# songhayeong/aes-fhe

Hardware: AMD Instinct MI355X
Metric: AES-128 blocks/sec (homomorphic full round) at N=2^16, L=30; 1/2/4/8 MI355X (higher is better)
Workload: dtype u64

## Files before the change

### aes-fhe_amd/csrc/engine.hip

```cpp
#include <hip/hip_runtime.h>

#include <algorithm>
#include <atomic>
#include <cstdarg>
#include <cstdlib>
#include <cstdio>
#include <cstring>
#include <map>
#include <unordered_map>
#include <memory>
#include <mutex>
#include <string>
#include <vector>

#include "../../include/aesfhe.h"
#include "kernels_ops.h"
#include "ntt256f.h"
#include "ks_fused.h"
#include "bconv_mfma.h"
#include "bconv_cols.h"
#include "basis_tables.h"
#include "bsgs_plan.h"
#include "operands.h"
#include "arena.h"
// ... 77 lines not shown
    }
    void split(void* p, int parts, size_t part) {
        if (!Arena::split(p, parts, part))
            throw_err(AESFHE_EARG, "pool split of a block that is not %d x %zu bytes", parts, part);
        if (trace) fprintf(trace, "s %c %p %d %zu\n", tag, p, parts, part);
    }
};

struct HipFree {
    void operator()(void* p) const { hipFree(p); }
};
struct DevBlocks {
    std::vector<std::unique_ptr<void, HipFree>> blocks;
    void* get(size_t bytes) {
        blocks.reserve(blocks.size() + 1);
        void* p = nullptr;
        HIPC(hipMalloc(&p, std::max<size_t>(bytes, 8)));
        blocks.emplace_back(p);
        return p;
    }
    template <typename T>
    T* up(const std::vector<T>& v) {
        T* d = (T*)get(v.size() * sizeof(T));
        HIPC(hipMemcpy(d, v.data(), v.size() * sizeof(T), hipMemcpyHostToDevice));
        return d;
    }
    void drop(void* p) {
        blocks.erase(std::remove_if(blocks.begin(), blocks.end(), [p](const auto& b) { return b.get() == p; }), blocks.end());
    }
};

struct ProfRec {
    int fam;
    hipEvent_t a, b;
    double bytes;
    const char* label;
    int disp;
};

struct KernStat {
    int64_t n = 0, d = 0;
    double ms = 0, bytes = 0;
};

struct MdTabs {
    const double *invf, *ninvf, *einv;
    const int8_t* tab;
    const double* corr;
    const u64* dinv;
    const double* dinvf;
    const TwD* hatf;
    const double* dmodf;
};

struct aesfhe_engine {
    std::atomic<int> refs{1};
    int logN, N, L, K, A, dnum, np, Lp1;
    int device = 0;
    u64 seed;
    ChaKey ck;
    Chain chain;
    hipStream_t stream = nullptr;
    Pool pool, tpool;
    size_t peak_total = 0;
    DevBlocks dev;
    u64* q;
    double* qinv;
    Tabs tab{};
    std::vector<u64> h_iroot;
    double *mu_hatinvf, *mu_nhatf, *rs_invf;
    MdTabs md;
    u64 *pmod, *rs_inv, *rs_mod;
    const double* pmodf;
    int8_t* bc_mu_tab;
    double *bc_mu_corr, *bc_pc;
    char* ring_d = nullptr;
    char* ring_h = nullptr;
    size_t ring_size = 8u << 20, ring_off = 0;
    double *ckre = nullptr, *ckim = nullptr;
    long* crot = nullptr;
    int* cflags = nullptr;
    size_t cflags_n = 0;
    std::map<std::string, TwD*> poly2_tabs;
    int prof = 0;
    std::vector<ProfRec> recs;
    std::vector<hipEvent_t> spare;
    double prof_ms[4] = {0, 0, 0, 0};
    double prof_bytes[4] = {0, 0, 0, 0};
    int64_t prof_n[4] = {0, 0, 0, 0};
    std::map<std::string, KernStat> prof_k;

    const Tabs& tabs() const { return tab; }

    ~aesfhe_engine() {
        if (!stream) return;
        hipSetDevice(device);
        hipStreamSynchronize(stream);
        for (auto& r : recs) {
            hipEventDestroy(r.a);
            hipEventDestroy(r.b);
        }
        for (auto ev : spare) hipEventDestroy(ev);
        pool.release_all();
        tpool.release_all();
        if (pool.trace) fclose(pool.trace);
        for (auto& kv : poly2_tabs) hipFree(kv.second);
        if (ring_d) hipFree(ring_d);
        if (ring_h) hipHostFree(ring_h);
        hipStreamDestroy(stream);
    }
};

struct aesfhe_key {
    aesfhe_engine* eng;
    int kind;
    u64 galois;
    u64 keyseed;
    u64* d;
    size_t bytes;
    int ndig = 0;
};

struct aesfhe_ct {
    aesfhe_engine* eng;
    int B, np, level, is_zero;
    u64* d;
    size_t bytes;
};

struct aesfhe_pt {
    aesfhe_engine* eng;
    int level;
    int ext = 0;
    u64* d;
    size_t bytes;
};

static const int FAM_NTT = 0, FAM_KS = 1, FAM_EW = 2;

struct ProfScope {
    aesfhe_engine* e;
    int fam;
    double bytes;
    hipEvent_t a = nullptr, b = nullptr;
    hipStream_t s;
    bool on;
    const char* label;
    int disp = 1;
    ProfScope(aesfhe_engine* e_, int f, double by, const char* lab = nullptr, hipStream_t s_ = nullptr)
        : e(e_), fam(f), bytes(by), s(s_ ? s_ : e_->stream), on((e_->prof >> f) & 1), label(lab) {
        if (!on) return;
        a = take();
        b = take();
        hipEventRecord(a, s);
    }
    hipEvent_t take() {
        if (!e->spare.empty()) {
            hipEvent_t x = e->spare.back();
            e->spare.pop_back();
            return x;
        }
        hipEvent_t x;
        hipEventCreate(&x);
        return x;
    }
    ~ProfScope() {
        if (!on) return;
        hipEventRecord(b, s);
        e->recs.push_back({fam, a, b, bytes, label, disp});
    }
};

static void prof_flush(aesfhe_engine* e) {
    if (e->recs.empty()) return;
    hipStreamSynchronize(e->stream);
    for (auto& r : e->recs) {
        float ms = 0;
        hipEventElapsedTime(&ms, r.a, r.b);
        e->prof_ms[r.fam] += ms;
        e->prof_bytes[r.fam] += r.bytes;
        e->prof_n[r.fam] += 1;
        if (r.label) {
            KernStat& k = e->prof_k[r.label];
            k.n++;
            k.d += r.disp;
            k.ms += ms;
            k.bytes += r.bytes;
        }
        e->spare.push_back(r.a);
// ... 2663 lines not shown
        const long obs = 3L * nl * N;
        d3 = ct_new(e, Bt, 3, l);
        {
            ProfScope ps_(e, FAM_EW, 8.0 * N * nl * (double)B * (2.0 * (nx + ny - 2) + 3.0 * ml), "poly2");
            for (int t0 = 0; t0 < ml; t0 += kPoly2Out)
                hipLaunchKernelGGL(k_poly2, ew_grid(e, nl, B), dim3(256), 0, e->stream, d[0].ptr, d[0].bs, d[0].ps, nx, d[1].ptr, d[1].bs, d[1].ps, ny, tab, ml, t0, std::min(kPoly2Out, ml - t0), d3->d, (long)B * obs, obs, e->q, e->qinv, e->logN);
        }
        HIPC(hipGetLastError());
    }
    poly2_finish(e, std::move(d3), rlk, live, m, B, l, outs);
    API_END
}

static void poly2_int_impl(aesfhe_engine* e, const aesfhe_ct* const* xb, int32_t nx, const aesfhe_ct* const* yb,
                           int32_t ny, const int32_t* w, int32_t den, int32_t m, const aesfhe_key* rlk,
                           aesfhe_ct** outs, int slab_rot);
extern "C" int aesfhe_poly2_int(aesfhe_engine* e, const aesfhe_ct* const* xb, int32_t nx, const aesfhe_ct* const* yb, int32_t ny, const int32_t* w, int32_t den, int32_t m, const aesfhe_key* rlk, aesfhe_ct** outs) {
    API_BEGIN
    poly2_int_impl(e, xb, nx, yb, ny, w, den, m, rlk, outs, 0);
    API_END
}
extern "C" int aesfhe_poly2_int_rot(aesfhe_engine* e, const aesfhe_ct* const* xb, int32_t nx, const aesfhe_ct* const* yb, int32_t ny, const int32_t* w, int32_t den, int32_t m, const aesfhe_key* rlk, int32_t slab_rot, aesfhe_ct** outs) {
    API_BEGIN
    if (slab_rot < 0 || slab_rot > 3) throw_err(AESFHE_EARG, "slab rotation %d outside 0..3", slab_rot);
    poly2_int_impl(e, xb, nx, yb, ny, w, den, m, rlk, outs, slab_rot);
    API_END
}
static void poly2_int_impl(aesfhe_engine* e, const aesfhe_ct* const* xb, int32_t nx, const aesfhe_ct* const* yb,
                           int32_t ny, const int32_t* w, int32_t den, int32_t m, const aesfhe_key* rlk,
                           aesfhe_ct** outs, int slab_rot) {
    const OperandScan sc = poly2_check(xb, nx, yb, ny, m, rlk, den);
    const int l = sc.level, B = sc.B;
    if (slab_rot && B % 4) throw_err(AESFHE_EARG, "slab rotation needs a batch of whole slabs (4 s), got %d", B);
    double wfac = 1.0;
    for (int t = 0; t < m; t++)
        for (int i = 0; i < nx; i++) {
            long sum = 0;
            double f = 0.0;
            for (int j = 0; j < ny; j++) {
                const long a = std::labs((long)w[((size_t)t * nx + i) * ny + j]);
                sum += a;
                f += j == 0 ? (double)a : 0.5 * (double)a + 1e-3 * (double)a;
            }
            if (sum > 512) throw_err(AESFHE_EARG, "poly2_int: sum of |w| over a row exceeds 512");
            wfac = std::max(wfac, f);
        }
    const int nl = l + 1, N = e->N;
    const double* D = e->chain.scale.data();
    const double S1 = D[l - 2] / D[l] * ((double)e->chain.q[l] / D[l]) * (double)e->chain.q[l - 1];
    const int64_t R = llround(D[l]);
    auto classes = [&](const aesfhe_ct* const* b, int n, std::vector<int>& cls, std::vector<int>& lev) {
        lev.clear();
        for (int i = 0; i < n - 1; i++)
            if (std::find(lev.begin(), lev.end(), b[i]->level) == lev.end()) lev.push_back(b[i]->level);
        std::sort(lev.rbegin(), lev.rend());
        cls.assign(n, 0);
        for (int i = 1; i < n; i++) cls[i] = 1 + (int)(std::find(lev.begin(), lev.end(), b[i - 1]->level) - lev.begin());
    };
    std::vector<int> cx, cy0, lx, ly;
    classes(xb, nx, cx, lx);
    classes(yb, ny, cy0, ly);
    std::vector<int> perm(ny), permx(nx);
    for (int j = 0; j < ny; j++) perm[j] = j;
    for (int i = 0; i < nx; i++) permx[i] = i;
    std::stable_sort(perm.begin() + 1, perm.end(), [&](int a, int b) { return cy0[a] < cy0[b]; });
    std::stable_sort(permx.begin() + 1, permx.end(), [&](int a, int b) { return cx[a] < cx[b]; });
    std::vector<int> cy(ny), cxs(nx);
    for (int j = 0; j < ny; j++) cy[j] = cy0[perm[j]];
    for (int i = 0; i < nx; i++) cxs[i] = cx[permx[i]];
    const int cxn = 1 + (int)lx.size(), cyn = 1 + (int)ly.size();
    std::vector<int> live;
    std::vector<double> Wt;
    for (int t = 0; t < m; t++) {
        bool any = false;
        for (size_t c = 0; c < (size_t)nx * ny; c++) any |= w[(size_t)t * nx * ny + c] != 0;
        if (!any) continue;
        live.push_back(t);
        for (int i = 0; i < nx; i++)
            for (int j = 0; j < ny; j++) Wt.push_back((double)w[((size_t)t * nx + permx[i]) * ny + perm[j]]);
    }
    const int ml = (int)live.size();
    CtPtr d3;
    if (ml > 0) {
        std::vector<TwD> Rt((size_t)nl * cxn * cyn);
        std::vector<double> C0((size_t)nl * cxn);
        for (int li = 0; li < nl; li++) {
            const u64 q = e->chain.q[li];
            const u64 r1 = h_smod(R, q);
            std::vector<u64> H((size_t)cxn * cyn);
            for (int a = 0; a < cxn; a++)
                for (int b = 0; b < cyn; b++) {
                    const double rx = a == 0 ? 1.0 : D[l] / D[lx[a - 1]];
                    const double ry = b == 0 ? 1.0 : D[l] / D[ly[b - 1]];
                    u64 h = h_smod(llround(S1 * rx * ry / (double)den), q);
                    if (a == 0) h = h_mulmod(h, r1, q);
                    if (b == 0) h = h_mulmod(h, r1, q);
                    H[(size_t)a * cyn + b] = h;
                }
            for (int a = 0; a < cxn; a++) {
                C0[(size_t)li * cxn + a] = (double)H[(size_t)a * cyn];
                for (int b = 0; b < cyn; b++) {
                    const u64 v = H[(size_t)a * cyn + b];
                    Rt[((size_t)li * cxn + a) * cyn + b] = TwD{(double)v, (double)v / (double)q};
                }
            }
        }
        const OperandTable tx = poly2_basis(xb, nx, permx.data(), B), ty = poly2_basis(yb, ny, perm.data(), B);
        const auto d = upload(e, {&tx, &ty}, OP_PTR | OP_BS | OP_PS);
        std::vector<int> xstart(cxn + 1, nx);
        for (int i = nx - 1; i >= 0; i--) xstart[cxs[i]] = i;
        auto dcx = upload_small(e, xstart.data(), xstart.size());
        auto dcy = upload_small(e, cy.data(), cy.size());
        auto dW = upload_small(e, Wt.data(), Wt.size());
        auto dR = upload_small(e, Rt.data(), Rt.size());
        auto dC0 = upload_small(e, C0.data(), C0.size());
        const long obs = 3L * nl * N;
        d3 = ct_new(e, ml * B, 3, l);
        auto is_big = [&](int li) {
            const double q = (double)e->chain.q[li];
            return wfac * q >= 0x1p52 * 0.999 || (wfac + 3.0 * nx) * q >= 0x1p53 * 0.999;
        };
        double wfac_u = 1.0;
        for (int t = 0; t < ml; t++)
            for (int i = 0; i < nx; i++) {
                double f = 0.0;
                for (int j = 0; j < ny; j++) f += std::fabs(Wt[((size_t)t * nx + i) * ny + j]);
                wfac_u = std::max(wfac_u, f);
            }
        auto lazy_ok = [&](int li) {
            const double q = (double)e->chain.q[li];
            return wfac_u * q < 0x1p51 && (wfac_u + 3.0 * nx) * q < 0x1p52;
        };
        {
            ProfScope ps_(e, FAM_EW, 8.0 * N * nl * (double)B * (2.0 * (nx + ny - 2) + 3.0 * ml), "poly2_int");
            ps_.disp = 0;
            constexpr int mo = 4;
            for (int t0 = 0; t0 < ml;) {
                const bool sbox = ny == kPoly2Max && ml - t0 >= 2 * mo && (N / 256) % 8 == 0;
                for (int la = 0; la < nl;) {
                    const bool big = is_big(la), lz = !big && lazy_ok(la);
                    int lb = la + 1;
                    while (lb < nl && is_big(lb) == big && (big || lazy_ok(lb) == lz)) lb++;
                    const dim3 grid(N / 256, lb - la, B);
                    bool split = big;
                    for (int li = la; li < lb; li++) split &= (double)e->chain.q[li] < 0x1p51;
                    if (sbox && split) {
                        hipLaunchKernelGGL(k_poly2_int_split<mo>, dim3(2 * N / 256, lb - la, B), dim3(256), 0, e->stream,
                                           d[0].ptr, d[0].bs, d[0].ps, nx, d[1].ptr, d[1].bs, d[1].ps,
                                           (const int*)dcx, (const int*)dcy, cxn, cyn, (const double*)dW, (const TwD*)dR, (const double*)dC0, t0,
                                           d3->d, (long)B * obs, obs, e->q, e->qinv, la, nl, e->logN, slab_rot);
                        ps_.disp++;
                    } else if (sbox) {
                        hipLaunchKernelGGL((big ? k_poly2_int_s<mo, false, true> : lz ? k_poly2_int_s<mo, true> : k_poly2_int_s<mo, false>), dim3(2 * N / 256, lb - la, B), dim3(256), 0, e->stream,
                                           d[0].ptr, d[0].bs, d[0].ps, nx, d[1].ptr, d[1].bs, d[1].ps,
                                           (const int*)dcx, (const int*)dcy, cxn, cyn, (const double*)dW, (const TwD*)dR, (const double*)dC0, t0,
                                           d3->d, (long)B * obs, obs, e->q, e->qinv, la, nl, e->logN, slab_rot);
                        ps_.disp++;
                    } else {
                        auto kern = big ? (ny == kPoly2Max ? k_poly2_int<true, kPoly2Max, mo> : k_poly2_int<true, 0, mo>)
                                        : (ny == kPoly2Max ? k_poly2_int<false, kPoly2Max, mo> : k_poly2_int<false, 0, mo>);
                        for (int tb = t0; tb < (sbox ? t0 + 2 * mo : t0 + mo) && tb < ml; tb += mo) {
                            hipLaunchKernelGGL(kern, grid, dim3(256), 0, e->stream, d[0].ptr, d[0].bs, d[0].ps, nx, d[1].ptr, d[1].bs, d[1].ps, ny,
                                               (const int*)dcx, (const int*)dcy, cxn, cyn, (const double*)dW, (const TwD*)dR, (const double*)dC0, ml, tb, std::min(mo, ml - tb), d3->d, (long)B * obs, obs, e->q, e->qinv, la, nl, e->logN, slab_rot);
                            ps_.disp++;
                        }
                    }
                    la = lb;
                }
                t0 += sbox ? 2 * mo : mo;
            }
        }
        HIPC(hipGetLastError());
    }
    poly2_finish(e, std::move(d3), rlk, live, m, B, l, outs);
}

extern "C" int aesfhe_ntt_host(aesfhe_engine* e, uint64_t* limbs, int32_t nlimb, const int32_t* pids, int32_t inv) {
    API_BEGIN
    const int N = e->N;
    for (int i = 0; i < nlimb; i++)
        if (pids[i] < 0 || pids[i] >= e->np) throw_err(AESFHE_EARG, "bad prime index");
    Tmp buf(e, (size_t)N);
    for (int i = 0; i < nlimb; i++) {
        HIPC(hipMemcpyAsync(buf.p, limbs + (size_t)i * N, (size_t)N * 8, hipMemcpyHostToDevice, e->stream));
        const int pid = pids[i];
        Span s = pid < e->Lp1 ? span_s(buf.p, N, 1, 1, pid, e->Lp1) : span_s(buf.p, N, 1, 0, 0, pid);
        ntt(e, s, s, 1, inv != 0);
        HIPC(hipMemcpyAsync(limbs + (size_t)i * N, buf.p, (size_t)N * 8, hipMemcpyDeviceToHost, e->stream));
        HIPC(hipStreamSynchronize(e->stream));
    }
    API_END
}

extern "C" int aesfhe_bench_ntt(aesfhe_engine* e, int32_t nlimb, int32_t iters, double* fwd_ms, double* inv_ms) {
    API_BEGIN
    const int N = e->N;
    const int nq = std::min(nlimb, e->Lp1);
    const int groups = (nlimb + nq - 1) / nq;
    Tmp buf(e, (size_t)groups * nq * N);
    HIPC(hipMemsetAsync(buf.p, 0, (size_t)groups * nq * N * 8, e->stream));
    Span s = span_s(buf.p, (long)nq * N, nq, nq, 0, e->Lp1);
    hipEvent_t a, b, c;
    HIPC(hipEventCreate(&a));
    HIPC(hipEventCreate(&b));
    HIPC(hipEventCreate(&c));
    ntt(e, s, s, groups * nq, false);
    ntt(e, s, s, groups * nq, true);
    HIPC(hipEventRecord(a, e->stream));
    for (int i = 0; i < iters; i++) ntt(e, s, s, groups * nq, false);
    HIPC(hipEventRecord(b, e->stream));
    for (int i = 0; i < iters; i++) ntt(e, s, s, groups * nq, true);
    HIPC(hipEventRecord(c, e->stream));
    HIPC(hipEventSynchronize(c));
    float t1 = 0, t2 = 0;
    hipEventElapsedTime(&t1, a, b);
    hipEventElapsedTime(&t2, b, c);
    *fwd_ms = t1 / iters;
    *inv_ms = t2 / iters;
    hipEventDestroy(a);
    hipEventDestroy(b);
    hipEventDestroy(c);
    API_END
}
```

### aes-fhe_amd/csrc/kernels_ops.h

```cpp
#pragma once
#include "kernels.h"

namespace aesfhe {

__device__ __forceinline__ u64 red_m(u64 x, u64 q, double qinv) {
    u64 qh = (u64)((double)x * qinv);
    return fix_m(x - qh * q, q);
}

struct Opnd {
    const u64* ptr;
    long bs;
    long ps;
    int np;
    int bmask = -1;
};

__device__ const u64 kZeroWord = 0;
__device__ __forceinline__ u64 opnd_get(const Opnd& o, int b, int p, int l, int k, int logN) {
    const bool has = o.ptr && p < o.np;
    return *(has ? o.ptr + (long)(b & o.bmask) * o.bs + (long)p * o.ps + ((long)l << logN) + k : &kZeroWord);
}

struct Out {
// ... 627 lines not shown
                        const long* __restrict__ ybs, const long* __restrict__ yps, int ny,
                        const TwD* __restrict__ F, int mtot, int t0, int mc,
                        u64* __restrict__ out, long oos, long obs, const u64* __restrict__ qs,
                        const double* __restrict__ qinv, int logN) {
    const int k = blockIdx.x * blockDim.x + threadIdx.x;
    const int l = blockIdx.y, bb = blockIdx.z, nl = gridDim.y;
    const int h = (int)((blockIdx.x * blockDim.x) >> (logN - 1));
    const double q = (double)qs[l];
    const double qi = qinv[l];
    const long off = ((long)l << logN) + k;
    double y0[kPoly2Max - 1], y1[kPoly2Max - 1];
#pragma unroll
    for (int j = 0; j < kPoly2Max - 1; j++) {
        y0[j] = y1[j] = 0.0;
        if (j < ny - 1) {
            const u64* p = yp[j] + (long)bb * ybs[j] + off;
            y0[j] = u2d(p[0]);
            y1[j] = u2d(p[yps[j]]);
        }
    }
    double d0[kPoly2Out], d1[kPoly2Out], d2[kPoly2Out];
#pragma unroll
    for (int t = 0; t < kPoly2Out; t++) d0[t] = d1[t] = d2[t] = 0.0;
    const TwD* Fl = F + ((size_t)(l * 2 + h) * mtot + t0) * nx * ny;
#pragma unroll 1
    for (int i = 0; i < nx; i++) {
        double xa = 0.0, xb = 0.0;
        if (i > 0) {
            const u64* p = xp[i - 1] + (long)bb * xbs[i - 1] + off;
            xa = u2d(p[0]);
            xb = u2d(p[xps[i - 1]]);
        }
#pragma unroll
        for (int t = 0; t < kPoly2Out; t++) {
            if (t < mc) {
                const TwD* Fi = Fl + ((size_t)t * nx + i) * ny;
                double a0 = Fi[0].w, a1 = 0.0;
#pragma unroll
                for (int j = 1; j < kPoly2Max; j++) {
                    if (j < ny) {
                        const TwD f = Fi[j];
                        a0 += fmul_rem_r(y0[j - 1], f.w, f.wq, q);
                        a1 += fmul_rem_r(y1[j - 1], f.w, f.wq, q);
                        if ((j & 3) == 0) {
                            a0 = fred(a0, q, qi);
                            a1 = fred(a1, q, qi);
                        }
                    }
                }
                a0 = fred(a0, q, qi);
                a1 = fred(a1, q, qi);
                if (i == 0) {
                    d0[t] += a0;
                    d1[t] += a1;
                } else {
                    const double a0q = a0 * qi, a1q = a1 * qi;
                    d0[t] += fmul_rem(xa, a0, a0q, q);
                    d1[t] += fmul_rem(xa, a1, a1q, q) + fmul_rem(xb, a0, a0q, q);
                    d2[t] += fmul_rem(xb, a1, a1q, q);
                }
                d0[t] = fred(d0[t], q, qi);
                d1[t] = fred(d1[t], q, qi);
                d2[t] = fred(d2[t], q, qi);
            }
        }
    }
    u64* o = out + (long)bb * obs + off;
    const long pstr = (long)nl << logN;
#pragma unroll
    for (int t = 0; t < kPoly2Out; t++) {
        if (t < mc) {
            u64* ot = o + (long)(t0 + t) * oos;
            ot[0] = fcanon(d0[t], q, qi);
            ot[pstr] = fcanon(d1[t], q, qi);
            ot[2 * pstr] = fcanon(d2[t], q, qi);
        }
    }
}

template <bool BIG, int NY, int MO>
__global__ void __launch_bounds__(256, MO > 4 ? 2 : 3) k_poly2_int(const u64* const* __restrict__ xp, const long* __restrict__ xbs,
                        const long* __restrict__ xps, int nx, const u64* const* __restrict__ yp,
                        const long* __restrict__ ybs, const long* __restrict__ yps, int ny,
                        const int* __restrict__ xstart, const int* __restrict__ ycls, int cxn,
                        int cyn, const double* __restrict__ Wt, const TwD* __restrict__ Rt,
                        const double* __restrict__ C0, int mtot, int t0, int mc,
                        u64* __restrict__ out, long oos, long obs, const u64* __restrict__ qs,
                        const double* __restrict__ qinv, int l0, int nl, int logN, int orot) {
    const int k = blockIdx.x * blockDim.x + threadIdx.x;
    const int l = l0 + blockIdx.y, bb = blockIdx.z;
    const double q = (double)qs[l];
    const double qi = qinv[l];
    constexpr bool big = BIG;
    const int nyv = NY > 0 ? NY : ny;
    const long off = ((long)l << logN) + k;
    double d0[MO], d1[MO], d2[MO];
#pragma unroll
    for (int t = 0; t < MO; t++) d0[t] = d1[t] = d2[t] = 0.0;
    const TwD* Rl = Rt + (size_t)l * cxn * cyn;
#pragma unroll 1
    for (int c = 0; c < cxn; c++) {
        const TwD* Rc = Rl + c * cyn;
        double y0[kPoly2Max - 1], y1[kPoly2Max - 1];
#pragma unroll
        for (int j = 0; j < kPoly2Max - 1; j++) {
            y0[j] = y1[j] = 0.0;
            if (j < nyv - 1) {
                const u64* p = yp[j] + (long)bb * ybs[j] + off;
                const TwD r = Rc[ycls[j + 1]];
                y0[j] = fred(fmul_rem_r(u2d(p[0]), r.w, r.wq, q), q, qi);
                y1[j] = fred(fmul_rem_r(u2d(p[yps[j]]), r.w, r.wq, q), q, qi);
            }
        }
        const double c0 = C0[(size_t)l * cxn + c];
#pragma unroll 1
    for (int i = xstart[c]; i < xstart[c + 1]; i++) {
        double xa = 0.0, xb = 0.0;
        if (i > 0) {
            const u64* p = xp[i - 1] + (long)bb * xbs[i - 1] + off;
            xa = u2d(p[0]);
            xb = u2d(p[xps[i - 1]]);
        }
#pragma unroll
        for (int t = 0; t < MO; t++) {
            if (t < mc) {
                const double* w = Wt + ((size_t)(t0 + t) * nx + i) * ny;
                double a0, a1;
                if constexpr (!big) {
                    a0 = w[0] * c0;
                    a1 = 0.0;
#pragma unroll
                    for (int j = 1; j < kPoly2Max; j++) {
                        if (j < nyv) {
                            a0 = __builtin_fma(w[j], y0[j - 1], a0);
                            a1 = __builtin_fma(w[j], y1[j - 1], a1);
                        }
                    }
                } else {
                    const double w0 = w[0];
                    a0 = fmul_rem(c0, w0, w0 * qi, q);
                    a1 = 0.0;
#pragma unroll
                    for (int j = 1; j < kPoly2Max; j++) {
                        if (j < nyv) {
                            const double wj = w[j], wjq = wj * qi;
                            a0 = fred(a0 + fmul_rem(y0[j - 1], wj, wjq, q), q, qi);
                            a1 = fred(a1 + fmul_rem(y1[j - 1], wj, wjq, q), q, qi);
                        }
                    }
                }
                if (i == 0) {
                    d0[t] += a0;
                    d1[t] += a1;
                } else {
                    const double a0q = a0 * qi, a1q = a1 * qi;
                    d0[t] += fmul_rem(xa, a0, a0q, q);
                    d1[t] += fmul_rem(xa, a1, a1q, q) + fmul_rem(xb, a0, a0q, q);
                    d2[t] += fmul_rem(xb, a1, a1q, q);
                }
                if constexpr (big) {
                    d0[t] = fred(d0[t], q, qi);
                    d1[t] = fred(d1[t], q, qi);
                    d2[t] = fred(d2[t], q, qi);
                }
            }
        }
    }
    }
    const int ob = (bb & ~3) | ((bb - orot) & 3);
    u64* o = out + (long)ob * obs + off;
    const long pstr = (long)nl << logN;
#pragma unroll
    for (int t = 0; t < MO; t++) {
        if (t < mc) {
            u64* ot = o + (long)(t0 + t) * oos;
            ot[0] = fcanon(d0[t], q, qi);
            ot[pstr] = fcanon(d1[t], q, qi);
            ot[2 * pstr] = fcanon(d2[t], q, qi);
        }
    }
}

template <int NY, bool BIG>
__device__ __forceinline__ void inner_sums(const double* __restrict__ w, double c0, const double (&y0)[NY - 1],
                                           const double (&y1)[NY - 1], double q, double qi, double& a0, double& a1) {
    if constexpr (!BIG) {
        a0 = w[0] * c0;
        a1 = 0.0;
#pragma unroll
        for (int j = 1; j < NY; j++) {
            a0 = __builtin_fma(w[j], y0[j - 1], a0);
            a1 = __builtin_fma(w[j], y1[j - 1], a1);
        }
    } else {
        const double w0 = w[0];
        a0 = fmul_rem(c0, w0, w0 * qi, q);
        a1 = 0.0;
#pragma unroll
        for (int j = 1; j < NY; j++) {
            const double wj = w[j], wjq = wj * qi;
            a0 = fred(a0 + fmul_rem(y0[j - 1], wj, wjq, q), q, qi);
            a1 = fred(a1 + fmul_rem(y1[j - 1], wj, wjq, q), q, qi);
        }
    }
}

template <int MO, bool LAZY, bool BIG = false>
__global__ void __launch_bounds__(256, 3) k_poly2_int_s(const u64* const* __restrict__ xp, const long* __restrict__ xbs,
                        const long* __restrict__ xps, int nx, const u64* const* __restrict__ yp,
                        const long* __restrict__ ybs, const long* __restrict__ yps,
                        const int* __restrict__ xstart, const int* __restrict__ ycls, int cxn,
                        int cyn, const double* __restrict__ Wt, const TwD* __restrict__ Rt,
                        const double* __restrict__ C0, int t0, u64* __restrict__ out, long oos, long obs,
                        const u64* __restrict__ qs, const double* __restrict__ qinv, int l0, int nl,
                        int logN, int orot) {
    constexpr int NY = kPoly2Max;
    static_assert(!(BIG && LAZY), "the folding path needs reduced y'");
    const int bx = blockIdx.x, half = (bx >> 3) & 1;
    const int k = (((bx >> 4) << 3) | (bx & 7)) * blockDim.x + threadIdx.x;
    const int l = l0 + blockIdx.y, bb = blockIdx.z;
    t0 += half * MO;
    const double q = (double)qs[l];
    const double qi = qinv[l];
    const long off = ((long)l << logN) + k;
    const TwD* Rl = Rt + (size_t)l * cxn * cyn;
    double y0[NY - 1], y1[NY - 1];
    auto load_y = [&](int c) {
        const TwD* Rc = Rl + c * cyn;
#pragma unroll
        for (int j = 0; j < NY - 1; j++) {
            const u64* p = yp[j] + (long)bb * ybs[j] + off;
            const TwD r = Rc[ycls[j + 1]];
            const double v0 = fmul_rem_r(u2d(p[0]), r.w, r.wq, q), v1 = fmul_rem_r(u2d(p[yps[j]]), r.w, r.wq, q);
            y0[j] = LAZY ? v0 : fred(v0, q, qi);
            y1[j] = LAZY ? v1 : fred(v1, q, qi);
        }
    };
    double d0[MO], d1[MO], d2[MO];
    load_y(0);
    {
        const double c0 = C0[(size_t)l * cxn];
#pragma unroll
        for (int t = 0; t < MO; t++) {
            const double* w = Wt + (size_t)(t0 + t) * nx * NY;
            double a0, a1;
            inner_sums<NY, BIG>(w, c0, y0, y1, q, qi, a0, a1);
            d0[t] = a0;
            d1[t] = a1;
            d2[t] = 0.0;
        }
    }
#pragma unroll 1
    for (int c = 1; c < cxn; c++) {
        load_y(c);
        const double c0 = C0[(size_t)l * cxn + c];
#pragma unroll 1
        for (int i = xstart[c]; i < xstart[c + 1]; i++) {
            const u64* p = xp[i - 1] + (long)bb * xbs[i - 1] + off;
            const double xa = u2d(p[0]), xb = u2d(p[xps[i - 1]]);
#pragma unroll
            for (int t = 0; t < MO; t++) {
                const double* w = Wt + ((size_t)(t0 + t) * nx + i) * NY;
                double a0, a1;
                inner_sums<NY, BIG>(w, c0, y0, y1, q, qi, a0, a1);
                const double a0q = a0 * qi, a1q = a1 * qi;
                d0[t] += fmul_rem(xa, a0, a0q, q);
                d1[t] += fmul_rem(xa, a1, a1q, q) + fmul_rem(xb, a0, a0q, q);
                d2[t] += fmul_rem(xb, a1, a1q, q);
                if constexpr (BIG) {
                    d0[t] = fred(d0[t], q, qi);
                    d1[t] = fred(d1[t], q, qi);
                    d2[t] = fred(d2[t], q, qi);
                }
            }
        }
    }
    const int ob = (bb & ~3) | ((bb - orot) & 3);
    u64* o = out + (long)ob * obs + off;
    const long pstr = (long)nl << logN;
#pragma unroll
    for (int t = 0; t < MO; t++) {
        u64* ot = o + (long)(t0 + t) * oos;
        ot[0] = fcanon(d0[t], q, qi);
        ot[pstr] = fcanon(d1[t], q, qi);
        ot[2 * pstr] = fcanon(d2[t], q, qi);
    }
}

template <int MO>
__global__ void __launch_bounds__(256, 3) k_poly2_int_split(const u64* const* __restrict__ xp, const long* __restrict__ xbs,
                        const long* __restrict__ xps, int nx, const u64* const* __restrict__ yp,
                        const long* __restrict__ ybs, const long* __restrict__ yps,
                        const int* __restrict__ xstart, const int* __restrict__ ycls, int cxn,
                        int cyn, const double* __restrict__ Wt, const TwD* __restrict__ Rt,
                        const double* __restrict__ C0, int t0, u64* __restrict__ out, long oos, long obs,
                        const u64* __restrict__ qs, const double* __restrict__ qinv, int l0, int nl,
                        int logN, int orot) {
    constexpr int NY = kPoly2Max;
    constexpr double S = 16777216.0, Si = 1.0 / 16777216.0;
    const int bx = blockIdx.x, half = (bx >> 3) & 1;
    const int k = (((bx >> 4) << 3) | (bx & 7)) * blockDim.x + threadIdx.x;
    const int l = l0 + blockIdx.y, bb = blockIdx.z;
    t0 += half * MO;
    const double q = (double)qs[l], qi = qinv[l], sq = S * qi;
    const long off = ((long)l << logN) + k;
    const TwD* Rl = Rt + (size_t)l * cxn * cyn;
    double d0[MO], d1[MO], d2[MO];
#pragma unroll
    for (int t = 0; t < MO; t++) d0[t] = d1[t] = d2[t] = 0.0;
#pragma unroll 1
    for (int p = 0; p < 2; p++) {
        double yh[NY - 1], yl[NY - 1];
#pragma unroll 1
        for (int c = 0; c < cxn; c++) {
            const TwD* Rc = Rl + c * cyn;
#pragma unroll
            for (int j = 0; j < NY - 1; j++) {
                const u64* yq = yp[j] + (long)bb * ybs[j] + off + (p ? yps[j] : 0);
                const TwD r = Rc[ycls[j + 1]];
                const double v = fred(fmul_rem_r(u2d(*yq), r.w, r.wq, q), q, qi);
                yh[j] = __builtin_rint(v * Si);
                yl[j] = __builtin_fma(-yh[j], S, v);
            }
            const double c0 = p ? 0.0 : C0[(size_t)l * cxn + c];
            const double c0h = __builtin_rint(c0 * Si), c0l = __builtin_fma(-c0h, S, c0);
#pragma unroll 1
            for (int i = xstart[c]; i < xstart[c + 1]; i++) {
                double xa = 1.0, xb = 0.0;
                if (i > 0) {
                    const u64* xq = xp[i - 1] + (long)bb * xbs[i - 1] + off;
                    xa = u2d(xq[0]);
                    xb = u2d(xq[xps[i - 1]]);
                }
#pragma unroll
                for (int t = 0; t < MO; t++) {
                    const double* w = Wt + ((size_t)(t0 + t) * nx + i) * NY;
                    double ah = w[0] * c0h, al = w[0] * c0l;
#pragma unroll
                    for (int j = 1; j < NY; j++) {
                        ah = __builtin_fma(w[j], yh[j - 1], ah);
                        al = __builtin_fma(w[j], yl[j - 1], al);
                    }
                    const double a = fmul_rem(ah, S, sq, q) + al, aq = a * qi;
                    if (i == 0) {
                        if (p == 0) d0[t] += a;
                        else d1[t] += a;
                    } else if (p == 0) {
                        d0[t] += fmul_rem(xa, a, aq, q);
                        d1[t] += fmul_rem(xb, a, aq, q);
                    } else {
                        d1[t] += fmul_rem(xa, a, aq, q);
                        d2[t] += fmul_rem(xb, a, aq, q);
                    }
                    d0[t] = fred(d0[t], q, qi);
                    d1[t] = fred(d1[t], q, qi);
                    d2[t] = fred(d2[t], q, qi);
                }
            }
        }
    }
    const int ob = (bb & ~3) | ((bb - orot) & 3);
    u64* o = out + (long)ob * obs + off;
    const long pstr = (long)nl << logN;
#pragma unroll
    for (int t = 0; t < MO; t++) {
        u64* ot = o + (long)(t0 + t) * oos;
        ot[0] = fcanon(d0[t], q, qi);
        ot[pstr] = fcanon(d1[t], q, qi);
        ot[2 * pstr] = fcanon(d2[t], q, qi);
    }
}

__global__ void k_lift0(const u64* __restrict__ x, u64* __restrict__ out, int nl, u64 q0,
                        const u64* __restrict__ qs, int logN) {
    const int k = blockIdx.x * blockDim.x + threadIdx.x;
    const int i = blockIdx.y, p = blockIdx.z;
    const u64 v = x[((long)p << logN) + k], q = qs[i];
    u64 r;
    if (v > (q0 >> 1)) {
        const u64 m = (q0 - v) % q;
        r = m ? q - m : 0;
    } else {
        r = v % q;
    }
    out[(((long)p * nl + i) << logN) + k] = r;
}

__global__ void k_dot_pt(const u64* const* __restrict__ cp, const long* __restrict__ cbs, long cps,
                         const u64* const* __restrict__ pp, int n, Out o, int np,
                         const u64* __restrict__ qs, const double* __restrict__ qinv, int logN) {
    const int k = blockIdx.x * blockDim.x + threadIdx.x;
    const int l = blockIdx.y, bb = blockIdx.z / np, p = blockIdx.z - bb * np;
    const double q = (double)qs[l], qi = qinv[l];
    const long off = ((long)l << logN) + k;
    double acc = 0.0;
    int i = 0;
    for (; i + 8 <= n; i += 8) {
        double cv[8], wv[8];
#pragma unroll
        for (int u = 0; u < 8; u++) {
            cv[u] = u2d(cp[i + u][(long)bb * cbs[i + u] + (long)p * cps + off]);
            wv[u] = u2d(pp[i + u][off]);
        }
#pragma unroll
        for (int u = 0; u < 8; u++) {
            acc += fmul_remq(cv[u], wv[u], qi, q);
            if ((u & 3) == 3) acc = fred(acc, q, qi);
        }
    }
    for (; i < n; i++) {
        const double c = u2d(cp[i][(long)bb * cbs[i] + (long)p * cps + off]);
        const double w = u2d(pp[i][off]);
        acc += fmul_remq(c, w, qi, q);
        if ((i & 3) == 3) acc = fred(acc, q, qi);
    }
    o.ptr[(long)bb * o.bs + (long)p * o.ps + off] = fcanon(acc, q, qi);
}

__device__ __forceinline__ int ext_pid(int t, int l, int Lp1) { return t <= l ? t : Lp1 + (t - l - 1); }

__global__ void k_scale_p_ext(Opnd in, u64* __restrict__ out, int l, int ne, const u64* __restrict__ qall,
                              const double* __restrict__ qinvall, const double* __restrict__ pmodf, int Lp1, int logN) {
    const int k = blockIdx.x * blockDim.x + threadIdx.x;
    const int t = blockIdx.y, bb = blockIdx.z >> 1, c = blockIdx.z & 1;
    u64 v = 0;
    if (t <= l) {
        const double q = (double)qall[t], qi = qinvall[t], f = pmodf[t];
        v = fcanon(fmul_rem(u2d(opnd_get(in, bb, c, t, k, logN)), tw_w(f, q), f, q), q, qi);
    }
    out[((((long)bb * 2 + c) * ne + t) << logN) + k] = v;
}

template <int GM, int BCT>
__global__ void k_dot_pt_ext_multi(const u64* const* __restrict__ ep, const u64* __restrict__ gal,
                                   const u64* const* __restrict__ pt, int nb,
// ... 206 lines not shown
```

Measured before the change: 286,600.

## Cache poly2 integer coefficient tables on device and simplify modular multiplies

```diff
diff --git a/aes-fhe_amd/csrc/engine.hip b/aes-fhe_amd/csrc/engine.hip
--- a/aes-fhe_amd/csrc/engine.hip
+++ b/aes-fhe_amd/csrc/engine.hip
@@ -183,6 +183,7 @@
     int* cflags = nullptr;
     size_t cflags_n = 0;
     std::map<std::string, TwD*> poly2_tabs;
+    std::map<std::string, void*> poly2_int_tabs;
     int prof = 0;
     std::vector<ProfRec> recs;
     std::vector<hipEvent_t> spare;
@@ -206,6 +207,7 @@
         tpool.release_all();
         if (pool.trace) fclose(pool.trace);
         for (auto& kv : poly2_tabs) hipFree(kv.second);
+        for (auto& kv : poly2_int_tabs) hipFree(kv.second);
         if (ring_d) hipFree(ring_d);
         if (ring_h) hipHostFree(ring_h);
         hipStreamDestroy(stream);
@@ -3035,43 +3037,59 @@
     const int ml = (int)live.size();
     CtPtr d3;
     if (ml > 0) {
-        std::vector<TwD> Rt((size_t)nl * cxn * cyn);
-        std::vector<double> C0((size_t)nl * cxn);
-        for (int li = 0; li < nl; li++) {
-            const u64 q = e->chain.q[li];
-            const u64 r1 = h_smod(R, q);
-            std::vector<u64> H((size_t)cxn * cyn);
-            for (int a = 0; a < cxn; a++)
-                for (int b = 0; b < cyn; b++) {
-                    const double rx = a == 0 ? 1.0 : D[l] / D[lx[a - 1]];
-                    const double ry = b == 0 ? 1.0 : D[l] / D[ly[b - 1]];
-                    u64 h = h_smod(llround(S1 * rx * ry / (double)den), q);
-                    if (a == 0) h = h_mulmod(h, r1, q);
-                    if (b == 0) h = h_mulmod(h, r1, q);
-                    H[(size_t)a * cyn + b] = h;
+        std::vector<int> xstart(cxn + 1, nx);
+        for (int i = nx - 1; i >= 0; i--) xstart[cxs[i]] = i;
+        const size_t nW = Wt.size(), nH = (size_t)nl * cxn * kPoly2Max;
+        const double* dW = nullptr;
+        {
+            const int hdr[7] = {l, nx, ny, den, m, cxn, cyn};
+            std::string key((const char*)hdr, sizeof hdr);
+            key.append((const char*)lx.data(), lx.size() * sizeof(int)).append((const char*)ly.data(), ly.size() * sizeof(int));
+            key.append((const char*)cx.data(), cx.size() * sizeof(int)).append((const char*)cy0.data(), cy0.size() * sizeof(int));
+            key.append((const char*)w, (size_t)m * nx * ny * sizeof(int32_t));
+            auto it = e->poly2_int_tabs.find(key);
+            if (it == e->poly2_int_tabs.end()) {
+                if (e->poly2_int_tabs.size() >= 64) {
+                    HIPC(hipStreamSynchronize(e->stream));
+                    for (auto& kv : e->poly2_int_tabs) HIPC(hipFree(kv.second));
+                    e->poly2_int_tabs.clear();
                 }
-            for (int a = 0; a < cxn; a++) {
-                C0[(size_t)li * cxn + a] = (double)H[(size_t)a * cyn];
-                for (int b = 0; b < cyn; b++) {
-                    const u64 v = H[(size_t)a * cyn + b];
-                    Rt[((size_t)li * cxn + a) * cyn + b] = TwD{(double)v, (double)v / (double)q};
+                std::vector<double> T(nW + nH + (xstart.size() + 1) / 2, 0.0);
+                std::copy(Wt.begin(), Wt.end(), T.begin());
+                for (int li = 0; li < nl; li++) {
+                    const u64 q = e->chain.q[li];
+                    const u64 r1 = h_smod(R, q);
+                    for (int a = 0; a < cxn; a++) {
+                        double* hc = T.data() + nW + ((size_t)li * cxn + a) * kPoly2Max;
+                        for (int b = 0; b < cyn; b++) {
+                            const double rx = a == 0 ? 1.0 : D[l] / D[lx[a - 1]];
+                            const double ry = b == 0 ? 1.0 : D[l] / D[ly[b - 1]];
+                            u64 h = h_smod(llround(S1 * rx * ry / (double)den), q);
+                            if (a == 0) h = h_mulmod(h, r1, q);
+                            if (b == 0) h = h_mulmod(h, r1, q);
+                            for (int j = 0; j < ny; j++)
+                                if (cy[j] == b) hc[j] = (double)h;
+                        }
+                    }
                 }
+                memcpy(T.data() + nW + nH, xstart.data(), xstart.size() * sizeof(int));
+                void* dT = nullptr;
+                HIPC(hipMalloc(&dT, T.size() * sizeof(double)));
+                HIPC(hipMemcpy(dT, T.data(), T.size() * sizeof(double), hipMemcpyHostToDevice));
+                it = e->poly2_int_tabs.emplace(std::move(key), dT).first;
             }
-        }
+            dW = (const double*)it->second;
+        }
+        const double* dH = dW + nW;
+        const int* dcx = (const int*)(dH + nH);
         const OperandTable tx = poly2_basis(xb, nx, permx.data(), B), ty = poly2_basis(yb, ny, perm.data(), B);
         const auto d = upload(e, {&tx, &ty}, OP_PTR | OP_BS | OP_PS);
-        std::vector<int> xstart(cxn + 1, nx);
-        for (int i = nx - 1; i >= 0; i--) xstart[cxs[i]] = i;
-        auto dcx = upload_small(e, xstart.data(), xstart.size());
-        auto dcy = upload_small(e, cy.data(), cy.size());
-        auto dW = upload_small(e, Wt.data(), Wt.size());
-        auto dR = upload_small(e, Rt.data(), Rt.size());
-        auto dC0 = upload_small(e, C0.data(), C0.size());
         const long obs = 3L * nl * N;
         d3 = ct_new(e, ml * B, 3, l);
         auto is_big = [&](int li) {
-            const double q = (double)e->chain.q[li];
-            return wfac * q >= 0x1p52 * 0.999 || (wfac + 3.0 * nx) * q >= 0x1p53 * 0.999;
+            const double q = (double)e->chain.q[li], A = wfac * q;
+            return A >= 0x1p52 * 0.999 || (wfac + 3.0 * nx) * q >= 0x1p53 * 0.999 ||
+                   A + 2.0 * (nx - 1) * (0.5 + 3.0 * 0x1p-53 * A * (1.0 + 0x1p-52)) * q >= 0x1p53 * 0.999;
         };
         double wfac_u = 1.0;
         for (int t = 0; t < ml; t++)
@@ -3100,13 +3118,13 @@
                     if (sbox && split) {
                         hipLaunchKernelGGL(k_poly2_int_split<mo>, dim3(2 * N / 256, lb - la, B), dim3(256), 0, e->stream,
                                            d[0].ptr, d[0].bs, d[0].ps, nx, d[1].ptr, d[1].bs, d[1].ps,
-                                           (const int*)dcx, (const int*)dcy, cxn, cyn, (const double*)dW, (const TwD*)dR, (const double*)dC0, t0,
+                                           dcx, cxn, dW, dH, t0,
                                            d3->d, (long)B * obs, obs, e->q, e->qinv, la, nl, e->logN, slab_rot);
                         ps_.disp++;
                     } else if (sbox) {
                         hipLaunchKernelGGL((big ? k_poly2_int_s<mo, false, true> : lz ? k_poly2_int_s<mo, true> : k_poly2_int_s<mo, false>), dim3(2 * N / 256, lb - la, B), dim3(256), 0, e->stream,
                                            d[0].ptr, d[0].bs, d[0].ps, nx, d[1].ptr, d[1].bs, d[1].ps,
-                                           (const int*)dcx, (const int*)dcy, cxn, cyn, (const double*)dW, (const TwD*)dR, (const double*)dC0, t0,
+                                           dcx, cxn, dW, dH, t0,
                                            d3->d, (long)B * obs, obs, e->q, e->qinv, la, nl, e->logN, slab_rot);
                         ps_.disp++;
                     } else {
@@ -3114,7 +3132,7 @@
                                         : (ny == kPoly2Max ? k_poly2_int<false, kPoly2Max, mo> : k_poly2_int<false, 0, mo>);
                         for (int tb = t0; tb < (sbox ? t0 + 2 * mo : t0 + mo) && tb < ml; tb += mo) {
                             hipLaunchKernelGGL(kern, grid, dim3(256), 0, e->stream, d[0].ptr, d[0].bs, d[0].ps, nx, d[1].ptr, d[1].bs, d[1].ps, ny,
-                                               (const int*)dcx, (const int*)dcy, cxn, cyn, (const double*)dW, (const TwD*)dR, (const double*)dC0, ml, tb, std::min(mo, ml - tb), d3->d, (long)B * obs, obs, e->q, e->qinv, la, nl, e->logN, slab_rot);
+                                               dcx, cxn, dW, dH, ml, tb, std::min(mo, ml - tb), d3->d, (long)B * obs, obs, e->q, e->qinv, la, nl, e->logN, slab_rot);
                             ps_.disp++;
                         }
                     }
diff --git a/aes-fhe_amd/csrc/kernels_ops.h b/aes-fhe_amd/csrc/kernels_ops.h
--- a/aes-fhe_amd/csrc/kernels_ops.h
+++ b/aes-fhe_amd/csrc/kernels_ops.h
@@ -733,9 +733,8 @@
 __global__ void __launch_bounds__(256, MO > 4 ? 2 : 3) k_poly2_int(const u64* const* __restrict__ xp, const long* __restrict__ xbs,
                         const long* __restrict__ xps, int nx, const u64* const* __restrict__ yp,
                         const long* __restrict__ ybs, const long* __restrict__ yps, int ny,
-                        const int* __restrict__ xstart, const int* __restrict__ ycls, int cxn,
-                        int cyn, const double* __restrict__ Wt, const TwD* __restrict__ Rt,
-                        const double* __restrict__ C0, int mtot, int t0, int mc,
+                        const int* __restrict__ xstart, int cxn, const double* __restrict__ Wt,
+                        const double* __restrict__ Hc, int mtot, int t0, int mc,
                         u64* __restrict__ out, long oos, long obs, const u64* __restrict__ qs,
                         const double* __restrict__ qinv, int l0, int nl, int logN, int orot) {
     const int k = blockIdx.x * blockDim.x + threadIdx.x;
@@ -748,22 +747,22 @@
     double d0[MO], d1[MO], d2[MO];
 #pragma unroll
     for (int t = 0; t < MO; t++) d0[t] = d1[t] = d2[t] = 0.0;
-    const TwD* Rl = Rt + (size_t)l * cxn * cyn;
+    const double* Hl = Hc + (size_t)l * cxn * kPoly2Max;
 #pragma unroll 1
     for (int c = 0; c < cxn; c++) {
-        const TwD* Rc = Rl + c * cyn;
+        const double* hc = Hl + c * kPoly2Max;
         double y0[kPoly2Max - 1], y1[kPoly2Max - 1];
 #pragma unroll
         for (int j = 0; j < kPoly2Max - 1; j++) {
             y0[j] = y1[j] = 0.0;
             if (j < nyv - 1) {
                 const u64* p = yp[j] + (long)bb * ybs[j] + off;
-                const TwD r = Rc[ycls[j + 1]];
-                y0[j] = fred(fmul_rem_r(u2d(p[0]), r.w, r.wq, q), q, qi);
-                y1[j] = fred(fmul_rem_r(u2d(p[yps[j]]), r.w, r.wq, q), q, qi);
-            }
-        }
-        const double c0 = C0[(size_t)l * cxn + c];
+                const double h = hc[j + 1];
+                y0[j] = fred(fmul_remq(u2d(p[0]), h, qi, q), q, qi);
+                y1[j] = fred(fmul_remq(u2d(p[yps[j]]), h, qi, q), q, qi);
+            }
+        }
+        const double c0 = hc[0];
 #pragma unroll 1
     for (int i = xstart[c]; i < xstart[c + 1]; i++) {
         double xa = 0.0, xb = 0.0;
@@ -788,15 +787,13 @@
                         }
                     }
                 } else {
-                    const double w0 = w[0];
-                    a0 = fmul_rem(c0, w0, w0 * qi, q);
+                    a0 = fmul_remq(c0, w[0], qi, q);
                     a1 = 0.0;
 #pragma unroll
                     for (int j = 1; j < kPoly2Max; j++) {
                         if (j < nyv) {
-                            const double wj = w[j], wjq = wj * qi;
-                            a0 = fred(a0 + fmul_rem(y0[j - 1], wj, wjq, q), q, qi);
-                            a1 = fred(a1 + fmul_rem(y1[j - 1], wj, wjq, q), q, qi);
+                            a0 = fred(a0 + fmul_remq(y0[j - 1], w[j], qi, q), q, qi);
+                            a1 = fred(a1 + fmul_remq(y1[j - 1], w[j], qi, q), q, qi);
                         }
                     }
                 }
@@ -804,10 +801,9 @@
                     d0[t] += a0;
                     d1[t] += a1;
                 } else {
-                    const double a0q = a0 * qi, a1q = a1 * qi;
-                    d0[t] += fmul_rem(xa, a0, a0q, q);
-                    d1[t] += fmul_rem(xa, a1, a1q, q) + fmul_rem(xb, a0, a0q, q);
-                    d2[t] += fmul_rem(xb, a1, a1q, q);
+                    d0[t] += fmul_remq(xa, a0, qi, q);
+                    d1[t] += fmul_remq(xa, a1, qi, q) + fmul_remq(xb, a0, qi, q);
+                    d2[t] += fmul_remq(xb, a1, qi, q);
                 }
                 if constexpr (big) {
                     d0[t] = fred(d0[t], q, qi);
@@ -844,14 +840,12 @@
             a1 = __builtin_fma(w[j], y1[j - 1], a1);
         }
     } else {
-        const double w0 = w[0];
-        a0 = fmul_rem(c0, w0, w0 * qi, q);
+        a0 = fmul_remq(c0, w[0], qi, q);
         a1 = 0.0;
 #pragma unroll
         for (int j = 1; j < NY; j++) {
-            const double wj = w[j], wjq = wj * qi;
-            a0 = fred(a0 + fmul_rem(y0[j - 1], wj, wjq, q), q, qi);
-            a1 = fred(a1 + fmul_rem(y1[j - 1], wj, wjq, q), q, qi);
+            a0 = fred(a0 + fmul_remq(y0[j - 1], w[j], qi, q), q, qi);
+            a1 = fred(a1 + fmul_remq(y1[j - 1], w[j], qi, q), q, qi);
         }
     }
 }
@@ -860,9 +854,8 @@
 __global__ void __launch_bounds__(256, 3) k_poly2_int_s(const u64* const* __restrict__ xp, const long* __restrict__ xbs,
                         const long* __restrict__ xps, int nx, const u64* const* __restrict__ yp,
                         const long* __restrict__ ybs, const long* __restrict__ yps,
-                        const int* __restrict__ xstart, const int* __restrict__ ycls, int cxn,
-                        int cyn, const double* __restrict__ Wt, const TwD* __restrict__ Rt,
-                        const double* __restrict__ C0, int t0, u64* __restrict__ out, long oos, long obs,
+                        const int* __restrict__ xstart, int cxn, const double* __restrict__ Wt,
+                        const double* __restrict__ Hc, int t0, u64* __restrict__ out, long oos, long obs,
                         const u64* __restrict__ qs, const double* __restrict__ qinv, int l0, int nl,
                         int logN, int orot) {
     constexpr int NY = kPoly2Max;
@@ -874,15 +867,15 @@
     const double q = (double)qs[l];
     const double qi = qinv[l];
     const long off = ((long)l << logN) + k;
-    const TwD* Rl = Rt + (size_t)l * cxn * cyn;
+    const double* Hl = Hc + (size_t)l * cxn * NY;
     double y0[NY - 1], y1[NY - 1];
     auto load_y = [&](int c) {
-        const TwD* Rc = Rl + c * cyn;
+        const double* hc = Hl + c * NY;
 #pragma unroll
         for (int j = 0; j < NY - 1; j++) {
             const u64* p = yp[j] + (long)bb * ybs[j] + off;
-            const TwD r = Rc[ycls[j + 1]];
-            const double v0 = fmul_rem_r(u2d(p[0]), r.w, r.wq, q), v1 = fmul_rem_r(u2d(p[yps[j]]), r.w, r.wq, q);
+            const double h = hc[j + 1];
+            const double v0 = fmul_remq(u2d(p[0]), h, qi, q), v1 = fmul_remq(u2d(p[yps[j]]), h, qi, q);
             y0[j] = LAZY ? v0 : fred(v0, q, qi);
             y1[j] = LAZY ? v1 : fred(v1, q, qi);
         }
@@ -890,7 +883,7 @@
     double d0[MO], d1[MO], d2[MO];
     load_y(0);
     {
-        const double c0 = C0[(size_t)l * cxn];
+        const double c0 = Hl[0];
 #pragma unroll
         for (int t = 0; t < MO; t++) {
             const double* w = Wt + (size_t)(t0 + t) * nx * NY;
@@ -904,7 +897,7 @@
 #pragma unroll 1
     for (int c = 1; c < cxn; c++) {
         load_y(c);
-        const double c0 = C0[(size_t)l * cxn + c];
+        const double c0 = Hl[c * NY];
 #pragma unroll 1
         for (int i = xstart[c]; i < xstart[c + 1]; i++) {
             const u64* p = xp[i - 1] + (long)bb * xbs[i - 1] + off;
@@ -914,10 +907,9 @@
                 const double* w = Wt + ((size_t)(t0 + t) * nx + i) * NY;
                 double a0, a1;
                 inner_sums<NY, BIG>(w, c0, y0, y1, q, qi, a0, a1);
-                const double a0q = a0 * qi, a1q = a1 * qi;
-                d0[t] += fmul_rem(xa, a0, a0q, q);
-                d1[t] += fmul_rem(xa, a1, a1q, q) + fmul_rem(xb, a0, a0q, q);
-                d2[t] += fmul_rem(xb, a1, a1q, q);
+                d0[t] += fmul_remq(xa, a0, qi, q);
+                d1[t] += fmul_remq(xa, a1, qi, q) + fmul_remq(xb, a0, qi, q);
+                d2[t] += fmul_remq(xb, a1, qi, q);
                 if constexpr (BIG) {
                     d0[t] = fred(d0[t], q, qi);
                     d1[t] = fred(d1[t], q, qi);
@@ -942,9 +934,8 @@
 __global__ void __launch_bounds__(256, 3) k_poly2_int_split(const u64* const* __restrict__ xp, const long* __restrict__ xbs,
                         const long* __restrict__ xps, int nx, const u64* const* __restrict__ yp,
                         const long* __restrict__ ybs, const long* __restrict__ yps,
-                        const int* __restrict__ xstart, const int* __restrict__ ycls, int cxn,
-                        int cyn, const double* __restrict__ Wt, const TwD* __restrict__ Rt,
-                        const double* __restrict__ C0, int t0, u64* __restrict__ out, long oos, long obs,
+                        const int* __restrict__ xstart, int cxn, const double* __restrict__ Wt,
+                        const double* __restrict__ Hc, int t0, u64* __restrict__ out, long oos, long obs,
                         const u64* __restrict__ qs, const double* __restrict__ qinv, int l0, int nl,
                         int logN, int orot) {
     constexpr int NY = kPoly2Max;
@@ -953,9 +944,9 @@
     const int k = (((bx >> 4) << 3) | (bx & 7)) * blockDim.x + threadIdx.x;
     const int l = l0 + blockIdx.y, bb = blockIdx.z;
     t0 += half * MO;
-    const double q = (double)qs[l], qi = qinv[l], sq = S * qi;
+    const double q = (double)qs[l], qi = qinv[l];
     const long off = ((long)l << logN) + k;
-    const TwD* Rl = Rt + (size_t)l * cxn * cyn;
+    const double* Hl = Hc + (size_t)l * cxn * NY;
     double d0[MO], d1[MO], d2[MO];
 #pragma unroll
     for (int t = 0; t < MO; t++) d0[t] = d1[t] = d2[t] = 0.0;
@@ -964,16 +955,15 @@
         double yh[NY - 1], yl[NY - 1];
 #pragma unroll 1
         for (int c = 0; c < cxn; c++) {
-            const TwD* Rc = Rl + c * cyn;
+            const double* hc = Hl + c * NY;
 #pragma unroll
             for (int j = 0; j < NY - 1; j++) {
                 const u64* yq = yp[j] + (long)bb * ybs[j] + off + (p ? yps[j] : 0);
-                const TwD r = Rc[ycls[j + 1]];
-                const double v = fred(fmul_rem_r(u2d(*yq), r.w, r.wq, q), q, qi);
+                const double v = fred(fmul_remq(u2d(*yq), hc[j + 1], qi, q), q, qi);
                 yh[j] = __builtin_rint(v * Si);
                 yl[j] = __builtin_fma(-yh[j], S, v);
             }
-            const double c0 = p ? 0.0 : C0[(size_t)l * cxn + c];
+            const double c0 = p ? 0.0 : hc[0];
             const double c0h = __builtin_rint(c0 * Si), c0l = __builtin_fma(-c0h, S, c0);
 #pragma unroll 1
             for (int i = xstart[c]; i < xstart[c + 1]; i++) {
@@ -992,16 +982,16 @@
                         ah = __builtin_fma(w[j], yh[j - 1], ah);
                         al = __builtin_fma(w[j], yl[j - 1], al);
                     }
-                    const double a = fmul_rem(ah, S, sq, q) + al, aq = a * qi;
+                    const double a = fmul_remq(ah, S, qi, q) + al;
                     if (i == 0) {
                         if (p == 0) d0[t] += a;
                         else d1[t] += a;
                     } else if (p == 0) {
-                        d0[t] += fmul_rem(xa, a, aq, q);
-                        d1[t] += fmul_rem(xb, a, aq, q);
+                        d0[t] += fmul_remq(xa, a, qi, q);
+                        d1[t] += fmul_remq(xb, a, qi, q);
                     } else {
-                        d1[t] += fmul_rem(xa, a, aq, q);
-                        d2[t] += fmul_rem(xb, a, aq, q);
+                        d1[t] += fmul_remq(xa, a, qi, q);
+                        d2[t] += fmul_remq(xb, a, qi, q);
                     }
                     d0[t] = fred(d0[t], q, qi);
                     d1[t] = fred(d1[t], q, qi);
```

New measurement: 288,100, median of 6. No clear change (+0.6%).
